# LordTARN1SHED/Image-Restoration-for-Road-Sign-Recognition-in-Autonomous-Driving

Hardware: AMD Instinct MI355X
Metric: images/sec ResUNet fwd+bwd (64x64 GTSRB batch) at 1/2/4/8 MI355X; PSNR parity (higher is better)
Workload: dtype bf16; 1 GPU; cfg3: ResUNet unified train step (dynamic distortion + ToTensor, fwd + L1 + 0.1*VGG16[:16] perceptual + bwd + AdamW), 14_train_unified_advanced.py; global_batch=512, per_gpu_batch=512, parallelism=dp1, hip_graph=True

## Files before the change

image-restoration-for-road-sign-recognition-in-autonomous-driving_amd/csrc/conv_in.hip:

```cpp
#include "common.h"

namespace {

template <typename T>
__global__ void conv_in_fwd_kernel(int n, int h, int w, int cin, int cout,
                                   const float *__restrict__ x, const float *__restrict__ wt,
                                   const float *__restrict__ b, int act, const float *alpha,
                                   T *__restrict__ y) {
  extern __shared__ __attribute__((aligned(16))) float sw[];
  const int kk = cin * 9;
  for (int i = threadIdx.x; i < kk * cout; i += blockDim.x) {
    const int co = i % cout, j = i / cout;
    sw[i] = wt[(long long)co * kk + j];
  }
  for (int i = threadIdx.x; i < cout; i += blockDim.x) sw[kk * cout + i] = b ? b[i] : 0.f;
  __syncthreads();
  const int G = cout / 4;
  const long long P = (long long)n * h * w;
  const float al = alpha ? alpha[0] : 0.f;
  for (long long id = blockIdx.x * (long long)blockDim.x + threadIdx.x; id < P * G;
       id += (long long)gridDim.x * blockDim.x) {
    const int g = (int)(id % G);
    const long long p = id / G;
    const int ww = (int)(p % w);
    const long long nh = p / w;
    const int hh = (int)(nh % h);
    const int nn = (int)(nh / h);
    f32x4 acc = *reinterpret_cast<const f32x4 *>(sw + kk * cout + g * 4);
    for (int ci = 0; ci < cin; ++ci) {
      const float *xp = x + ((long long)nn * cin + ci) * h * w;
#pragma unroll
      for (int t = 0; t < 9; ++t) {
        const int y2 = hh + t / 3 - 1, x2 = ww + t % 3 - 1;
        if (y2 < 0 || y2 >= h || x2 < 0 || x2 >= w) continue;
        const float v = xp[(long long)y2 * w + x2];
        acc += v * *reinterpret_cast<const f32x4 *>(sw + (ci * 9 + t) * cout + g * 4);
      }
    }
    if (act == 1) {
#pragma unroll
      for (int k = 0; k < 4; ++k) acc[k] = fmaxf(acc[k], 0.f);
    } else if (act == 2) {
#pragma unroll
      for (int k = 0; k < 4; ++k) acc[k] = acc[k] > 0.f ? acc[k] : al * acc[k];
    }
    store4<T>(y + p * cout + g * 4, acc);
  }
}

template <typename T>
__global__ void conv_in_wgrad_kernel(int n, int h, int w, int cin, int cout,
                                     const float *__restrict__ x, const T *__restrict__ dy,
                                     float *__restrict__ part, long long px_per_block) {
  __shared__ __attribute__((aligned(16))) float sdy[64][65];
  __shared__ __attribute__((aligned(16))) float spt[64][32];
  const int kk = cin * 9;
  const long long P = (long long)n * h * w;
  const long long pb = blockIdx.x * px_per_block;
  const long long pe = min(P, pb + px_per_block);
  const int co = threadIdx.x & 63, jg = threadIdx.x >> 6;
  double acc[8] = {0, 0, 0, 0, 0, 0, 0, 0};
  for (long long p0 = pb; p0 < pe; p0 += 64) {
    __syncthreads();
    for (int i = threadIdx.x; i < 64 * 64; i += blockDim.x) {
      const int r = i >> 6, c = i & 63;
      const long long p = p0 + r;
      sdy[r][c] = (p < pe && c < cout) ? Elt<T>::load(dy, p * cout + c) : 0.f;
    }
    for (int i = threadIdx.x; i < 64 * 32; i += blockDim.x) {
      const int r = i >> 5, j = i & 31;
      const long long p = p0 + r;
      float v = 0.f;
      if (p < pe) {
        if (j < kk) {
          const int ci = j / 9, t = j % 9;
          const int ww = (int)(p % w);
          const long long nh = p / w;
          const int hh = (int)(nh % h);
          const int nn = (int)(nh / h);
          const int y2 = hh + t / 3 - 1, x2 = ww + t % 3 - 1;
          if (y2 >= 0 && y2 < h && x2 >= 0 && x2 < w)
            v = x[(((long long)nn * cin + ci) * h + y2) * w + x2];
        } else if (j == kk) {
          v = 1.f;
        }
      }
      spt[r][j] = v;
    }
    __syncthreads();
    if (co < cout) {
      float st[8] = {0.f, 0.f, 0.f, 0.f, 0.f, 0.f, 0.f, 0.f};
#pragma unroll 4
      for (int r = 0; r < 64; ++r) {
        const float d = sdy[r][co];
        const f32x4 a0 = *reinterpret_cast<const f32x4 *>(&spt[r][jg * 8]);
        const f32x4 a1 = *reinterpret_cast<const f32x4 *>(&spt[r][jg * 8 + 4]);
#pragma unroll
        for (int k = 0; k < 4; ++k) { st[k] += d * a0[k]; st[4 + k] += d * a1[k]; }
      }
#pragma unroll
      for (int k = 0; k < 8; ++k) acc[k] += st[k];
    }
  }
  if (co < cout) {
#pragma unroll
    for (int k = 0; k < 8; ++k) part[((long long)blockIdx.x * cout + co) * 32 + jg * 8 + k] = (float)acc[k];
  }
}

constexpr int CIA_NPX = 64;
constexpr int CIA_ROW = CIA_NPX + 8;
constexpr int CIA_XROW = 32 + 8;
template <bool REC>
__global__ __launch_bounds__(256, REC ? 4 : 1) void conv_in_wgrad_act_kernel(
    int n, int h, int w, const float *__restrict__ x, const bf16_t *__restrict__ g,
    const bf16_t *__restrict__ t, int act, const float *__restrict__ alpha,
    float *__restrict__ part, long long ppb) {
  __shared__ __attribute__((aligned(16))) u16 gT[64 * CIA_ROW];
  __shared__ __attribute__((aligned(16))) u16 pT[32 * CIA_ROW];
  __shared__ __attribute__((aligned(16))) u16 pX[REC ? CIA_NPX * CIA_XROW : 8];
  __shared__ float red[256];
  const int tid = threadIdx.x, lane = tid & 63, wv = tid >> 6;
  const long long P = (long long)n * h * w, hw = (long long)h * w;
  const long long p0 = blockIdx.x * ppb, p1 = min(P, p0 + ppb);
  const float al = act == 2 ? alpha[0] : 0.f;
  float sa = 0.f;
  f32x4 acc[2] = {f32x4{0.f, 0.f, 0.f, 0.f}, f32x4{0.f, 0.f, 0.f, 0.f}};
  const int lc = tid & 7, lpp = tid >> 3;
  const int bn = lane & 15, bk = lane >> 4;
  const int sj = tid & 63, sg = tid >> 6;
  uint4 rg[2], rt[2] = {};
  float rp[8];
  auto load_step = [&](long long q0) __attribute__((always_inline)) {
#pragma unroll
    for (int j = 0; j < 2; ++j) {
      const long long p = q0 + 2 * lpp + j;
      const bool ok = p < p1;
      const long long e = (ok ? p : p0) * 64 + lc * 8;
      rg[j] = *reinterpret_cast<const uint4 *>(g + e);
      if constexpr (!REC) rt[j] = *reinterpret_cast<const uint4 *>(t + e);
      if (!ok) rg[j] = uint4{0u, 0u, 0u, 0u};
    }
    const long long p = q0 + sj;
    const bool live = p < p1;
    int img = 0, y = 0, xx0 = 0;
    if (live) {
      img = (int)(p / hw);
      const int rem = (int)(p - img * hw);
      y = rem / w;
      xx0 = rem - y * w;
    }
#pragma unroll
    for (int u = 0; u < 8; ++u) {
      const int r = sg + 4 * u;
      float val = 0.f;
      if (r < 27) {
        const int ci = r / 9, ky = (r % 9) / 3, kx = r % 3;
        const int yy = y + ky - 1, xx = xx0 + kx - 1;
        const bool ok = live && yy >= 0 && yy < h && xx >= 0 && xx < w;
        const float vv = x[ok ? (((long long)img * 3 + ci) * h + yy) * w + xx : 0];
        val = ok ? vv : 0.f;
      } else if (r == 27) {
        val = live ? 1.f : 0.f;
      }
      rp[u] = val;
    }
  };
  auto bf = [](uint32_t word, int hi) { return __uint_as_float(hi ? (word & 0xffff0000u) : (word << 16)); };
  bf16x8 fw = {};
  if constexpr (REC) fw = *reinterpret_cast<const bf16x8 *>(t + (wv * 16 + bn) * 32 + bk * 8);
  if (p0 < p1) load_step(p0);
  for (long long q0 = p0; q0 < p1; q0 += CIA_NPX) {
    if constexpr (REC) {
#pragma unroll
      for (int u = 0; u < 8; ++u) {
        const u16 pv = f32_to_bf16(rp[u]);
        pT[(sg + 4 * u) * CIA_ROW + sj] = pv;
        pX[sj * CIA_XROW + sg + 4 * u] = pv;
      }
      __syncthreads();
#pragma unroll
      for (int nb = 0; nb < 4; ++nb) {
        const bf16x8 fp = *reinterpret_cast<const bf16x8 *>(&pX[(nb * 16 + bn) * CIA_XROW + bk * 8]);
        const f32x4 tv = __builtin_amdgcn_mfma_f32_16x16x32_bf16(fw, fp, f32x4{0.f, 0.f, 0.f, 0.f}, 0, 0, 0);
#pragma unroll
        for (int i = 0; i < 4; ++i) gT[(wv * 16 + 4 * bk + i) * CIA_ROW + nb * 16 + bn] = f32_to_bf16(tv[i]);
      }
      __syncthreads();
    }
    u16 v[2][8];
    uint32_t tpair[8];
    if constexpr (REC) {
#pragma unroll
      for (int k = 0; k < 8; ++k)
        tpair[k] = *reinterpret_cast<const uint32_t *>(&gT[(lc * 8 + k) * CIA_ROW + 2 * lpp]);
    }
#pragma unroll
    for (int j = 0; j < 2; ++j) {
      const uint32_t gw[4] = {rg[j].x, rg[j].y, rg[j].z, rg[j].w};
      const uint32_t tw[4] = {rt[j].x, rt[j].y, rt[j].z, rt[j].w};
#pragma unroll
      for (int k = 0; k < 8; ++k) {
        const float gg = bf(gw[k >> 1], k & 1);
        const float tt = REC ? bf(tpair[k], j) : bf(tw[k >> 1], k & 1);
        const float gp = tt > 0.f ? gg : al * gg;
        sa += tt > 0.f ? 0.f : gg * tt;
        v[j][k] = f32_to_bf16(gp);
      }
    }
#pragma unroll
    for (int k = 0; k < 8; ++k)
      *reinterpret_cast<uint32_t *>(&gT[(lc * 8 + k) * CIA_ROW + 2 * lpp]) =
          (uint32_t)v[0][k] | ((uint32_t)v[1][k] << 16);
    if constexpr (!REC) {
#pragma unroll
      for (int u = 0; u < 8; ++u) pT[(sg + 4 * u) * CIA_ROW + sj] = f32_to_bf16(rp[u]);
    }
    __syncthreads();
    if (q0 + CIA_NPX < p1) load_step(q0 + CIA_NPX);
#pragma unroll
    for (int ks = 0; ks < 2; ++ks) {
      const int px = ks * 32 + bk * 8;
      const bf16x8 fa = *reinterpret_cast<const bf16x8 *>(&gT[(wv * 16 + bn) * CIA_ROW + px]);
#pragma unroll
      for (int nb = 0; nb < 2; ++nb) {
        const bf16x8 fb = *reinterpret_cast<const bf16x8 *>(&pT[(nb * 16 + bn) * CIA_ROW + px]);
        acc[nb] = __builtin_amdgcn_mfma_f32_16x16x32_bf16(fa, fb, acc[nb], 0, 0, 0);
      }
    }
    __syncthreads();
  }
  float *pw = part + (long long)blockIdx.x * (64 * 32 + 32);
#pragma unroll
  for (int nb = 0; nb < 2; ++nb)
#pragma unroll
    for (int i = 0; i < 4; ++i) pw[(wv * 16 + 4 * bk + i) * 32 + nb * 16 + bn] = acc[nb][i];
  red[tid] = sa;
  __syncthreads();
  for (int o = 128; o > 0; o >>= 1) {
    if (tid < o) red[tid] += red[tid + o];
    __syncthreads();
  }
  if (tid < 32) pw[64 * 32 + tid] = tid == 0 ? red[0] : 0.f;
}

__global__ void conv_in_wgrad_act_finalize(int chunks, const double *__restrict__ part, float *dw,
                                           float *db, float *dalpha) {
  const int i = blockIdx.x * blockDim.x + threadIdx.x;
  const int cols = 64 * 32 + 32;
  if (i > 64 * 32) return;
  double sv[1] = {0};
  rr_fixed_sum<1>(part + i, cols, chunks, sv);
  const double s = sv[0];
  if (i == 64 * 32) {
    if (dalpha) dalpha[0] = (float)s;
    return;
  }
  const int co = i / 32, j = i % 32;
  if (j < 27) dw[co * 27 + j] = (float)s;
  else if (j == 27 && db) db[co] = (float)s;
}

__global__ void conv_in_wgrad_finalize(int cout, int kk, int blocks, const double *__restrict__ part,
                                       float *dw, float *db) {
  const int i = blockIdx.x * blockDim.x + threadIdx.x;
  if (i >= cout * 32) return;
  const int co = i / 32, j = i % 32;
  if (j > kk) return;
  double sv[1] = {0};
  rr_fixed_sum<1>(part + i, (long long)cout * 32, blocks, sv);
  const double s = sv[0];
  if (j < kk) dw[(long long)co * kk + j] = (float)s;
  else if (db) db[co] = (float)s;
}

template <typename T>
__global__ void conv_in_dgrad_kernel(int n, int h, int w, int cin, int cout,
                                     const T *__restrict__ dy, const float *__restrict__ wt,
                                     float *__restrict__ dx, int accumulate) {
  extern __shared__ __attribute__((aligned(16))) float sw[];
  const int kk = cin * 9;
  for (int i = threadIdx.x; i < kk * cout; i += blockDim.x) {
    const int co = i % cout, j = i / cout;
    const int t = j / cin, ci = j % cin;
    sw[i] = wt[((long long)co * cin + ci) * 9 + t];
  }
  __syncthreads();
  const long long P = (long long)n * h * w;
  for (long long p = blockIdx.x * (long long)blockDim.x + threadIdx.x; p < P;
       p += (long long)gridDim.x * blockDim.x) {
    const int ww = (int)(p % w);
    const long long nh = p / w;
    const int hh = (int)(nh % h);
    const int nn = (int)(nh / h);
    float acc[4] = {0.f, 0.f, 0.f, 0.f};
    for (int t = 0; t < 9; ++t) {
      const int ky = t / 3, kx = t % 3;
      const int y2 = hh - ky + 1, x2 = ww - kx + 1;
      if (y2 < 0 || y2 >= h || x2 < 0 || x2 >= w) continue;
      const T *dp = dy + (((long long)nn * h + y2) * w + x2) * cout;
      for (int c = 0; c < cout; c += 4) {
        const f32x4 d = load4<T>(dp + c);
        for (int ci = 0; ci < cin && ci < 4; ++ci) {
          const f32x4 wv = *reinterpret_cast<const f32x4 *>(sw + (t * cin + ci) * cout + c);
          acc[ci] += d[0] * wv[0] + d[1] * wv[1] + d[2] * wv[2] + d[3] * wv[3];
        }
      }
    }
    for (int ci = 0; ci < cin && ci < 4; ++ci) {
      const long long o = (((long long)nn * cin + ci) * h + hh) * w + ww;
      dx[o] = accumulate ? dx[o] + acc[ci] : acc[ci];
    }
  }
}

template <typename T>
__global__ void im2col3_kernel(int n, int h, int w, int cin, int kpad, const float *__restrict__ x,
                               T *__restrict__ col) {
  const int G = kpad / 4;
  const long long total = (long long)n * h * w * G;
  const int kk = cin * 9;
  for (long long i = blockIdx.x * (long long)blockDim.x + threadIdx.x; i < total;
       i += (long long)gridDim.x * blockDim.x) {
    const int g = (int)(i % G);
    const long long p = i / G;
    const int ww = (int)(p % w);
    const long long nh = p / w;
    const int hh = (int)(nh % h);
    const int nn = (int)(nh / h);
    f32x4 v;
#pragma unroll
    for (int e = 0; e < 4; ++e) {
      const int j = g * 4 + e;
      float val = 0.f;
      if (j < kk) {
        const int ci = j / 9, t = j - (j / 9) * 9;
        const int y2 = hh + t / 3 - 1, x2 = ww + t % 3 - 1;
        if (y2 >= 0 && y2 < h && x2 >= 0 && x2 < w)
          val = x[(((long long)nn * cin + ci) * h + y2) * w + x2];
      } else if (j == kk) {
        val = 1.f;
      }
      v[e] = val;
    }
    store4<T>(col + p * kpad + g * 4, v);
  }
}

__global__ __launch_bounds__(256) void conv_in_mfma_kernel(int n, int h, int w,
                                                           const float *__restrict__ x,
                                                           const bf16_t *__restrict__ wp, int act,
                                                           const float *__restrict__ alpha,
                                                           bf16_t *__restrict__ y_pre,
                                                           bf16_t *__restrict__ y_act) {
  constexpr int SR = 68;
  __shared__ __attribute__((aligned(16))) float stg[4][32 * SR];
  const int lane = threadIdx.x & 63, wv = threadIdx.x >> 6;
  const long long hw = (long long)h * w;
  const long long P = (long long)n * hw;
  const long long p0 = ((long long)blockIdx.x * 4 + wv) * 64;
  if (p0 >= P) return;
  const int fr = lane & 15, q = lane >> 4;
  bf16x8 fa[4];
#pragma unroll
  for (int mi = 0; mi < 4; ++mi)
    fa[mi] = *reinterpret_cast<const bf16x8 *>(wp + (mi * 16 + fr) * 32 + q * 8);
  const int hwi = h * w;
  int kofs[8], kdy[8], kdx[8];
  bool ktap[8], kone[8];
#pragma unroll
  for (int j = 0; j < 8; ++j) {
    const int k = q * 8 + j;
    const int ci = k / 9, t = k - (k / 9) * 9;
    kdy[j] = t / 3 - 1;
    kdx[j] = t % 3 - 1;
    kofs[j] = ci * hwi + kdy[j] * w + kdx[j];
    ktap[j] = k < 27;
    kone[j] = k == 27;
  }
  const int Pi = (int)P;
  const __amdgpu_buffer_rsrc_t xr = __builtin_amdgcn_make_buffer_rsrc(
      const_cast<float *>(x), 0, (int)(3 * P * 4), 0x00020000);
  const int pw0 = (int)p0;
// ... 217 lines not shown
```

image-restoration-for-road-sign-recognition-in-autonomous-driving_amd/csrc/conv_out.hip:

```cpp
#include "common.h"

namespace {

template <typename T>
__global__ void conv_out_fwd_kernel(int n, int h, int w, int cin, int cout, const T *__restrict__ x,
                                    const float *__restrict__ wt, const float *__restrict__ b,
                                    float *__restrict__ y) {
  extern __shared__ __attribute__((aligned(16))) float sw[];
  for (int i = threadIdx.x; i < cin * cout; i += blockDim.x) sw[i] = wt[i];
  __syncthreads();
  const long long P = (long long)n * h * w;
  const long long hw = (long long)h * w;
  for (long long p = blockIdx.x * (long long)blockDim.x + threadIdx.x; p < P;
       p += (long long)gridDim.x * blockDim.x) {
    float acc[4] = {0.f, 0.f, 0.f, 0.f};
    const T *xp = x + p * cin;
    for (int c = 0; c < cin; c += 4) {
      const f32x4 v = load4<T>(xp + c);
      for (int co = 0; co < cout && co < 4; ++co) {
        const f32x4 wv = *reinterpret_cast<const f32x4 *>(sw + co * cin + c);
        acc[co] += v[0] * wv[0] + v[1] * wv[1] + v[2] * wv[2] + v[3] * wv[3];
      }
    }
    const long long nn = p / hw, r = p % hw;
    for (int co = 0; co < cout && co < 4; ++co)
      y[(nn * cout + co) * hw + r] = acc[co] + (b ? b[co] : 0.f);
  }
}

template <typename T>
__global__ void conv_out_bwd_kernel(int n, int h, int w, int cin, int cout,
                                    const float *__restrict__ dy, const T *__restrict__ x,
                                    const float *__restrict__ wt, T *__restrict__ dx, int mask_relu,
                                    float *__restrict__ part, long long px_per_block) {
  __shared__ float red[4][64][4];
  __shared__ float redb[4][4];
  const int ci = threadIdx.x & 63, row = threadIdx.x >> 6;
  const long long hw = (long long)h * w;
  const long long P = (long long)n * hw;
  const long long pb = blockIdx.x * px_per_block;
  const long long pe = min(P, pb + px_per_block);
  float wv[4] = {0.f, 0.f, 0.f, 0.f};
  for (int co = 0; co < cout; ++co) wv[co] = ci < cin ? wt[co * cin + ci] : 0.f;
  float sw[4] = {0.f, 0.f, 0.f, 0.f}, sb[4] = {0.f, 0.f, 0.f, 0.f};
  for (long long p = pb + row; p < pe; p += 4) {
    const long long nn = p / hw, r = p - nn * hw;
    float d[4] = {0.f, 0.f, 0.f, 0.f};
    for (int co = 0; co < cout; ++co) d[co] = dy[(nn * cout + co) * hw + r];
    if (ci < cin) {
      const float xv = Elt<T>::load(x, p * cin + ci);
      float g = 0.f;
      for (int co = 0; co < cout; ++co) {
        g += d[co] * wv[co];
        sw[co] += d[co] * xv;
      }
      if (mask_relu && !(xv > 0.f)) g = 0.f;
      if (dx) Elt<T>::store(dx, p * cin + ci, g);
    }
    for (int co = 0; co < cout; ++co) sb[co] += d[co];
  }
  for (int co = 0; co < 4; ++co) red[row][ci][co] = sw[co];
  if (ci == 0)
    for (int co = 0; co < 4; ++co) redb[row][co] = sb[co];
  __syncthreads();
  if (row == 0 && ci < cin)
    for (int co = 0; co < cout; ++co)
      part[((long long)blockIdx.x * (cout + 1) + co) * cin + ci] =
          red[0][ci][co] + red[1][ci][co] + red[2][ci][co] + red[3][ci][co];
  if (threadIdx.x < cout) {
    const int co = threadIdx.x;
    part[((long long)blockIdx.x * (cout + 1) + cout) * cin + co] =
        redb[0][co] + redb[1][co] + redb[2][co] + redb[3][co];
  }
}

template <typename T, int COUT>
__global__ __launch_bounds__(256) void conv_out_bwd64_kernel(
    int n, int h, int w, const float *__restrict__ dy, const T *__restrict__ x,
    const float *__restrict__ wt, T *__restrict__ dx, int mask_relu, float *__restrict__ part,
    long long px_per_block) {
  constexpr int CIN = 64;
  __shared__ float red[4][COUT + 1][CIN];
  const int cg = threadIdx.x & 7, pl = threadIdx.x >> 3;
  const long long hw = (long long)h * w;
  const long long P = (long long)n * hw;
  const long long pb = blockIdx.x * px_per_block;
  const long long pe = min(P, pb + px_per_block);
  float wv[COUT][8];
#pragma unroll
  for (int co = 0; co < COUT; ++co)
#pragma unroll
    for (int j = 0; j < 8; ++j) wv[co][j] = wt[co * CIN + cg * 8 + j];
  float sw[COUT][8], sb[COUT];
#pragma unroll
  for (int co = 0; co < COUT; ++co) {
    sb[co] = 0.f;
#pragma unroll
    for (int j = 0; j < 8; ++j) sw[co][j] = 0.f;
  }
  auto one = [&](long long p) __attribute__((always_inline)) {
    const long long nn = p / hw, r = p - nn * hw;
    float d[COUT];
#pragma unroll
    for (int co = 0; co < COUT; ++co) d[co] = dy[(nn * COUT + co) * hw + r];
    const T *xp = x + p * CIN + cg * 8;
    const f32x4 x0 = load4<T>(xp), x1 = load4<T>(xp + 4);
    const float xv[8] = {x0[0], x0[1], x0[2], x0[3], x1[0], x1[1], x1[2], x1[3]};
    float g[8];
#pragma unroll
    for (int j = 0; j < 8; ++j) {
      float t = 0.f;
#pragma unroll
      for (int co = 0; co < COUT; ++co) {
        t += d[co] * wv[co][j];
        sw[co][j] += d[co] * xv[j];
      }
      g[j] = (mask_relu && !(xv[j] > 0.f)) ? 0.f : t;
    }
#pragma unroll
    for (int co = 0; co < COUT; ++co) sb[co] += d[co];
    if (dx) store8<T>(dx + p * CIN + cg * 8, f32x4{g[0], g[1], g[2], g[3]}, f32x4{g[4], g[5], g[6], g[7]});
  };
  long long p = pb + pl;
  for (; p + 32 < pe; p += 64) {
    one(p);
    one(p + 32);
  }
  if (p < pe) one(p);
#pragma unroll
  for (int co = 0; co < COUT; ++co) {
#pragma unroll
    for (int j = 0; j < 8; ++j) {
      float v = sw[co][j];
      v += __shfl_xor(v, 8, 64);
      v += __shfl_xor(v, 16, 64);
      v += __shfl_xor(v, 32, 64);
      sw[co][j] = v;
    }
    float v = sb[co];
    v += __shfl_xor(v, 8, 64);
    v += __shfl_xor(v, 16, 64);
    v += __shfl_xor(v, 32, 64);
    sb[co] = v;
  }
  const int wv_ = threadIdx.x >> 6, lane = threadIdx.x & 63;
  if (lane < 8) {
#pragma unroll
    for (int co = 0; co < COUT; ++co) {
#pragma unroll
      for (int j = 0; j < 8; ++j) red[wv_][co][cg * 8 + j] = sw[co][j];
      if (cg == 0) red[wv_][COUT][co] = sb[co];
    }
  }
  __syncthreads();
  for (int i = threadIdx.x; i < COUT * CIN + COUT; i += 256) {
    const int co = i / CIN, ci = i - co * CIN;
    part[(long long)blockIdx.x * (COUT + 1) * CIN + i] =
        red[0][co][ci] + red[1][co][ci] + red[2][co][ci] + red[3][co][ci];
  }
}

template <typename T, int COUT, bool REC = false>
__global__ __launch_bounds__(256) void conv_out_bwd64_bnred_kernel(
    int n, int h, int w, const float *__restrict__ dy, const T *__restrict__ x,
    const float *__restrict__ wt, const T *__restrict__ t0, const float *__restrict__ mean0,
    const float *__restrict__ inv0, const T *__restrict__ t1, const float *__restrict__ mean1,
    const float *__restrict__ inv1, float *__restrict__ part, float *__restrict__ bnpart,
    long long px_per_block, const float *__restrict__ aff_s = nullptr,
    const float *__restrict__ aff_b = nullptr) {
  constexpr int CIN = 64;
  __shared__ float red[4][COUT + 1][CIN];
  __shared__ float bred[4][CIN][3];
  const int cg = threadIdx.x & 7, pl = threadIdx.x >> 3;
  const long long hw = (long long)h * w;
  const long long P = (long long)n * hw;
  const long long pb = blockIdx.x * px_per_block;
  const long long pe = min(P, pb + px_per_block);
  float wv[COUT][8], m0[8], i0[8], m1[8], i1[8];
#pragma unroll
  for (int j = 0; j < 8; ++j) {
#pragma unroll
    for (int co = 0; co < COUT; ++co) wv[co][j] = wt[co * CIN + cg * 8 + j];
    m0[j] = mean0[cg * 8 + j]; i0[j] = inv0[cg * 8 + j];
    m1[j] = mean1[cg * 8 + j]; i1[j] = inv1[cg * 8 + j];
  }
  __shared__ __attribute__((aligned(16))) float faff[REC ? 4 * CIN : 4];
  if constexpr (REC) {
    faff[threadIdx.x] = threadIdx.x < 2 * CIN ? aff_s[threadIdx.x] : aff_b[threadIdx.x - 2 * CIN];
    __syncthreads();
  }
  float sw[COUT][8], sb[COUT], bs[3][8];
#pragma unroll
  for (int co = 0; co < COUT; ++co) {
    sb[co] = 0.f;
#pragma unroll
    for (int j = 0; j < 8; ++j) sw[co][j] = 0.f;
  }
#pragma unroll
  for (int j = 0; j < 8; ++j) { bs[0][j] = 0.f; bs[1][j] = 0.f; bs[2][j] = 0.f; }
  auto one = [&](long long p) __attribute__((always_inline)) {
    const long long nn = p / hw, r = p - nn * hw;
    float d[COUT];
#pragma unroll
    for (int co = 0; co < COUT; ++co) d[co] = dy[(nn * COUT + co) * hw + r];
    const long long e = p * CIN + cg * 8;
    f32x4 x0, x1, a0, a1, b0, b1;
    load8<T>(t0 + e, a0, a1);
    load8<T>(t1 + e, b0, b1);
    if constexpr (REC) {
      int o = cg * 8;
      asm volatile("" : "+v"(o));
      const f32x4 *fa = reinterpret_cast<const f32x4 *>(faff + o);
      f32x4 v0 = a0 * fa[0] + fa[32], v1 = a1 * fa[1] + fa[33];
      f32x4 q0 = b0 * fa[16] + fa[48], q1 = b1 * fa[17] + fa[49];
      v0 += q0;
      v1 += q1;
#pragma unroll
      for (int k = 0; k < 4; ++k) {
        x0[k] = Elt<T>::round(fmaxf(v0[k], 0.f));
        x1[k] = Elt<T>::round(fmaxf(v1[k], 0.f));
      }
    } else {
      load8<T>(x + e, x0, x1);
    }
    const float xv[8] = {x0[0], x0[1], x0[2], x0[3], x1[0], x1[1], x1[2], x1[3]};
    const float ta[8] = {a0[0], a0[1], a0[2], a0[3], a1[0], a1[1], a1[2], a1[3]};
    const float tb[8] = {b0[0], b0[1], b0[2], b0[3], b1[0], b1[1], b1[2], b1[3]};
#pragma unroll
    for (int j = 0; j < 8; ++j) {
      float t = 0.f;
#pragma unroll
      for (int co = 0; co < COUT; ++co) {
        t += d[co] * wv[co][j];
        sw[co][j] += d[co] * xv[j];
      }
      const float gm = xv[j] > 0.f ? Elt<T>::round(t) : 0.f;
      bs[0][j] += gm;
      bs[1][j] += gm * ((ta[j] - m0[j]) * i0[j]);
      bs[2][j] += gm * ((tb[j] - m1[j]) * i1[j]);
    }
#pragma unroll
    for (int co = 0; co < COUT; ++co) sb[co] += d[co];
  };
  long long p = pb + pl;
  for (; p + 32 < pe; p += 64) {
    one(p);
    one(p + 32);
  }
  if (p < pe) one(p);
  auto lanes8 = [](float v) __attribute__((always_inline)) {
    v += __shfl_xor(v, 8, 64);
    v += __shfl_xor(v, 16, 64);
    v += __shfl_xor(v, 32, 64);
    return v;
  };
#pragma unroll
  for (int co = 0; co < COUT; ++co) {
#pragma unroll
    for (int j = 0; j < 8; ++j) sw[co][j] = lanes8(sw[co][j]);
    sb[co] = lanes8(sb[co]);
  }
#pragma unroll
  for (int k = 0; k < 3; ++k)
#pragma unroll
    for (int j = 0; j < 8; ++j) bs[k][j] = lanes8(bs[k][j]);
  const int wv_ = threadIdx.x >> 6, lane = threadIdx.x & 63;
  if (lane < 8) {
#pragma unroll
    for (int co = 0; co < COUT; ++co) {
#pragma unroll
      for (int j = 0; j < 8; ++j) red[wv_][co][cg * 8 + j] = sw[co][j];
      if (cg == 0) red[wv_][COUT][co] = sb[co];
    }
#pragma unroll
    for (int j = 0; j < 8; ++j)
#pragma unroll
      for (int k = 0; k < 3; ++k) bred[wv_][cg * 8 + j][k] = bs[k][j];
  }
  __syncthreads();
  for (int i = threadIdx.x; i < COUT * CIN + COUT; i += 256) {
    const int co = i / CIN, ci = i - co * CIN;
    part[(long long)blockIdx.x * (COUT + 1) * CIN + i] =
        red[0][co][ci] + red[1][co][ci] + red[2][co][ci] + red[3][co][ci];
  }
  if (threadIdx.x < CIN * 3) {
    const int c = threadIdx.x / 3, k = threadIdx.x - c * 3;
    bnpart[(long long)blockIdx.x * CIN * 3 + threadIdx.x] =
        bred[0][c][k] + bred[1][c][k] + bred[2][c][k] + bred[3][c][k];
  }
}

constexpr int TCO_D = 2;
__global__ __launch_bounds__(256) void tail_conv_out_kernel(
    int P, int hw, int cout, const bf16_t *__restrict__ x, const float *__restrict__ scale,
    const float *__restrict__ shift, const bf16_t *__restrict__ res, const float *__restrict__ rs,
    const float *__restrict__ rb, const bf16_t *__restrict__ wp, const float *__restrict__ bias,
    bf16_t *__restrict__ y, float *__restrict__ out) {
  const int lane = threadIdx.x & 63;
  const int wv = __builtin_amdgcn_readfirstlane(threadIdx.x >> 6);
  const int fr = lane & 15, fq = lane >> 4;
  const int nblk = (P + 15) >> 4;
  const int gw = blockIdx.x * 4 + wv, NWT = gridDim.x * 4;
  bf16x8 wr[2];
  f32x4 s[2][2], b[2][2], qs[2][2], qb[2][2];
#pragma unroll
  for (int kb = 0; kb < 2; ++kb) {
    bf16x8 v = {};
    if (fr < cout) v = *reinterpret_cast<const bf16x8 *>(wp + fr * 64 + kb * 32 + fq * 8);
    wr[kb] = v;
#pragma unroll
    for (int hf = 0; hf < 2; ++hf) {
      const int c = kb * 32 + fq * 8 + 4 * hf;
      s[kb][hf] = *reinterpret_cast<const f32x4 *>(scale + c);
      b[kb][hf] = *reinterpret_cast<const f32x4 *>(shift + c);
      qs[kb][hf] = *reinterpret_cast<const f32x4 *>(rs + c);
      qb[kb][hf] = *reinterpret_cast<const f32x4 *>(rb + c);
    }
  }
  float bv[4];
#pragma unroll
  for (int j = 0; j < 4; ++j) bv[j] = j < cout ? bias[j] : 0.f;
  struct Blk {
    uint4 t[2], r[2];
  };
  auto load_blk = [&](int bi, Blk &bk) __attribute__((always_inline)) {
    const int p = min(bi * 16 + fr, P - 1);
    const long long e = (long long)p * 64 + fq * 8;
#pragma unroll
    for (int kb = 0; kb < 2; ++kb) {
      bk.t[kb] = *reinterpret_cast<const uint4 *>(x + e + kb * 32);
      bk.r[kb] = *reinterpret_cast<const uint4 *>(res + e + kb * 32);
    }
  };
  auto unpack = [](uint4 r, f32x4 &lo, f32x4 &hi) __attribute__((always_inline)) {
    lo[0] = __uint_as_float(r.x << 16); lo[1] = __uint_as_float(r.x & 0xffff0000u);
    lo[2] = __uint_as_float(r.y << 16); lo[3] = __uint_as_float(r.y & 0xffff0000u);
    hi[0] = __uint_as_float(r.z << 16); hi[1] = __uint_as_float(r.z & 0xffff0000u);
    hi[2] = __uint_as_float(r.w << 16); hi[3] = __uint_as_float(r.w & 0xffff0000u);
  };
  auto run = [&](const Blk &bk, int bi) __attribute__((always_inline)) {
    const int p = bi * 16 + fr;
    const bool live = p < P;
    f32x4 acc = f32x4{0.f, 0.f, 0.f, 0.f};
#pragma unroll
    for (int kb = 0; kb < 2; ++kb) {
      f32x4 v0, v1, q0, q1;
      unpack(bk.t[kb], v0, v1);
      unpack(bk.r[kb], q0, q1);
      v0 = v0 * s[kb][0] + b[kb][0];
      v1 = v1 * s[kb][1] + b[kb][1];
      q0 = q0 * qs[kb][0] + qb[kb][0];
      q1 = q1 * qs[kb][1] + qb[kb][1];
      v0 += q0;
      v1 += q1;
#pragma unroll
      for (int k = 0; k < 4; ++k) { v0[k] = fmaxf(v0[k], 0.f); v1[k] = fmaxf(v1[k], 0.f); }
      u16x8 r;
      r[0] = f32_to_bf16(v0[0]); r[1] = f32_to_bf16(v0[1]); r[2] = f32_to_bf16(v0[2]); r[3] = f32_to_bf16(v0[3]);
      r[4] = f32_to_bf16(v1[0]); r[5] = f32_to_bf16(v1[1]); r[6] = f32_to_bf16(v1[2]); r[7] = f32_to_bf16(v1[3]);
      if (y && live) *reinterpret_cast<u16x8 *>(y + (long long)p * 64 + kb * 32 + fq * 8) = r;
      acc = __builtin_amdgcn_mfma_f32_16x16x32_bf16(wr[kb], __builtin_bit_cast(bf16x8, r), acc, 0, 0, 0);
    }
    if (live && fq == 0) {
      const int n = p / hw, rem = p - n * hw;
#pragma unroll
      for (int j = 0; j < 4; ++j)
        if (j < cout) out[((long long)n * cout + j) * hw + rem] = acc[j] + bv[j];
    }
  };
  for (int b0 = gw; b0 < nblk; b0 += TCO_D * NWT) {
    Blk bk[TCO_D];
#pragma unroll
    for (int j = 0; j < TCO_D; ++j) load_blk(min(b0 + j * NWT, nblk - 1), bk[j]);
#pragma unroll
    for (int j = 0; j < TCO_D; ++j)
      if (b0 + j * NWT < nblk) run(bk[j], b0 + j * NWT);
  }
}

__global__ void conv_out_bwd_finalize(int cin, int cout, int blocks, const double *__restrict__ part,
                                      float *dw, float *db) {
  const int i = blockIdx.x * blockDim.x + threadIdx.x;
  if (i >= cout * cin + cout) return;
  double s = 0;
  if (i < cout * cin) {
    double sv[1] = {0};
    rr_fixed_sum<1>(part + i, (long long)(cout + 1) * cin, blocks, sv);
    s = sv[0];
    if (dw) dw[i] = (float)s;
  } else {
    const int co = i - cout * cin;
    double sv[1] = {0};
    rr_fixed_sum<1>(part + (long long)cout * cin + co, (long long)(cout + 1) * cin, blocks, sv);
    s = sv[0];
    if (db) db[co] = (float)s;
  }
}

}

extern "C" int rr_conv_out_fwd(int dtype, int n, int h, int w, int cin, int cout, const void *x,
                               const float *wt, const float *b, float *y, rr_stream stream) {
// ... 153 lines not shown
```

Baseline: 36940 images/sec.

## Double-buffer conv_in wgrad LDS tiles and software-prefetch conv_out bwd pixel loads

The first-layer weight-gradient kernel now gives each thread one pixel. It recomputes the fused activation input in registers with MFMA instead of staging it through an extra LDS array, and it replaces per-step div/mod with an incremental position walker. The gT/pT tiles are double-buffered, which drops one barrier per iteration, and launch bounds are raised to 4 waves for both variants. In conv_out backward, loads for the next two pixels are issued before the current ones are used, and an incremental plane walker replaces the per-pixel division. The changes trade more registers and LDS for better latency hiding, and the MFMA operand remapping must exactly match the previous layout.

```diff
diff --git a/image-restoration-for-road-sign-recognition-in-autonomous-driving_amd/csrc/conv_in.hip b/image-restoration-for-road-sign-recognition-in-autonomous-driving_amd/csrc/conv_in.hip
--- a/image-restoration-for-road-sign-recognition-in-autonomous-driving_amd/csrc/conv_in.hip
+++ b/image-restoration-for-road-sign-recognition-in-autonomous-driving_amd/csrc/conv_in.hip
@@ -110,15 +110,13 @@
 
 constexpr int CIA_NPX = 64;
 constexpr int CIA_ROW = CIA_NPX + 8;
-constexpr int CIA_XROW = 32 + 8;
 template <bool REC>
-__global__ __launch_bounds__(256, REC ? 4 : 1) void conv_in_wgrad_act_kernel(
+__global__ __launch_bounds__(256, 4) void conv_in_wgrad_act_kernel(
     int n, int h, int w, const float *__restrict__ x, const bf16_t *__restrict__ g,
     const bf16_t *__restrict__ t, int act, const float *__restrict__ alpha,
     float *__restrict__ part, long long ppb) {
-  __shared__ __attribute__((aligned(16))) u16 gT[64 * CIA_ROW];
-  __shared__ __attribute__((aligned(16))) u16 pT[32 * CIA_ROW];
-  __shared__ __attribute__((aligned(16))) u16 pX[REC ? CIA_NPX * CIA_XROW : 8];
+  __shared__ __attribute__((aligned(16))) u16 gT[2][64 * CIA_ROW];
+  __shared__ __attribute__((aligned(16))) u16 pT[2][32 * CIA_ROW];
   __shared__ float red[256];
   const int tid = threadIdx.x, lane = tid & 63, wv = tid >> 6;
   const long long P = (long long)n * h * w, hw = (long long)h * w;
@@ -126,109 +124,114 @@
   const float al = act == 2 ? alpha[0] : 0.f;
   float sa = 0.f;
   f32x4 acc[2] = {f32x4{0.f, 0.f, 0.f, 0.f}, f32x4{0.f, 0.f, 0.f, 0.f}};
-  const int lc = tid & 7, lpp = tid >> 3;
   const int bn = lane & 15, bk = lane >> 4;
-  const int sj = tid & 63, sg = tid >> 6;
+  const int px = wv * 16 + bn;
+  long long kofs[8];
+  int kdy[8], kdx[8];
+  bool ktap[8], kone[8];
+#pragma unroll
+  for (int j = 0; j < 8; ++j) {
+    const int k = bk * 8 + j;
+    const int ci = k / 9, tp = k - ci * 9;
+    kdy[j] = tp / 3 - 1;
+    kdx[j] = tp % 3 - 1;
+    kofs[j] = ci * hw + kdy[j] * (long long)w + kdx[j];
+    ktap[j] = k < 27;
+    kone[j] = k == 27;
+  }
+  long long pq = p0 + px, xo = 0;
+  int py = 0, pxx = 0;
+  if (pq < p1) {
+    const long long img = pq / hw;
+    const int rem = (int)(pq - img * hw);
+    py = rem / w;
+    pxx = rem - py * w;
+    xo = img * 3 * hw + rem;
+  }
+  auto next_pos = [&]() __attribute__((always_inline)) {
+    pq += CIA_NPX;
+    xo += CIA_NPX;
+    pxx += CIA_NPX;
+    while (pxx >= w) {
+      pxx -= w;
+      if (++py == h) { py = 0; xo += 2 * hw; }
+    }
+  };
   uint4 rg[2], rt[2] = {};
   float rp[8];
-  auto load_step = [&](long long q0) __attribute__((always_inline)) {
-#pragma unroll
-    for (int j = 0; j < 2; ++j) {
-      const long long p = q0 + 2 * lpp + j;
-      const bool ok = p < p1;
-      const long long e = (ok ? p : p0) * 64 + lc * 8;
-      rg[j] = *reinterpret_cast<const uint4 *>(g + e);
-      if constexpr (!REC) rt[j] = *reinterpret_cast<const uint4 *>(t + e);
-      if (!ok) rg[j] = uint4{0u, 0u, 0u, 0u};
-    }
-    const long long p = q0 + sj;
-    const bool live = p < p1;
-    int img = 0, y = 0, xx0 = 0;
-    if (live) {
-      img = (int)(p / hw);
-      const int rem = (int)(p - img * hw);
-      y = rem / w;
-      xx0 = rem - y * w;
-    }
-#pragma unroll
-    for (int u = 0; u < 8; ++u) {
-      const int r = sg + 4 * u;
-      float val = 0.f;
-      if (r < 27) {
-        const int ci = r / 9, ky = (r % 9) / 3, kx = r % 3;
-        const int yy = y + ky - 1, xx = xx0 + kx - 1;
-        const bool ok = live && yy >= 0 && yy < h && xx >= 0 && xx < w;
-        const float vv = x[ok ? (((long long)img * 3 + ci) * h + yy) * w + xx : 0];
-        val = ok ? vv : 0.f;
-      } else if (r == 27) {
-        val = live ? 1.f : 0.f;
-      }
-      rp[u] = val;
+  auto load_step = [&]() __attribute__((always_inline)) {
+    const bool live = pq < p1;
+    const long long e = (live ? pq : p0) * 64 + bk * 8;
+#pragma unroll
+    for (int c = 0; c < 2; ++c) {
+      rg[c] = *reinterpret_cast<const uint4 *>(g + e + c * 32);
+      if constexpr (!REC) rt[c] = *reinterpret_cast<const uint4 *>(t + e + c * 32);
+      if (!live) rg[c] = uint4{0u, 0u, 0u, 0u};
+    }
+#pragma unroll
+    for (int j = 0; j < 8; ++j) {
+      const int yy = py + kdy[j], xx = pxx + kdx[j];
+      const bool ok = live && ktap[j] && (unsigned)yy < (unsigned)h && (unsigned)xx < (unsigned)w;
+      const float vv = x[ok ? xo + kofs[j] : 0];
+      rp[j] = ok ? vv : (kone[j] && live ? 1.f : 0.f);
     }
   };
   auto bf = [](uint32_t word, int hi) { return __uint_as_float(hi ? (word & 0xffff0000u) : (word << 16)); };
-  bf16x8 fw = {};
-  if constexpr (REC) fw = *reinterpret_cast<const bf16x8 *>(t + (wv * 16 + bn) * 32 + bk * 8);
-  if (p0 < p1) load_step(p0);
-  for (long long q0 = p0; q0 < p1; q0 += CIA_NPX) {
-    if constexpr (REC) {
-#pragma unroll
-      for (int u = 0; u < 8; ++u) {
-        const u16 pv = f32_to_bf16(rp[u]);
-        pT[(sg + 4 * u) * CIA_ROW + sj] = pv;
-        pX[sj * CIA_XROW + sg + 4 * u] = pv;
-      }
-      __syncthreads();
-#pragma unroll
-      for (int nb = 0; nb < 4; ++nb) {
-        const bf16x8 fp = *reinterpret_cast<const bf16x8 *>(&pX[(nb * 16 + bn) * CIA_XROW + bk * 8]);
-        const f32x4 tv = __builtin_amdgcn_mfma_f32_16x16x32_bf16(fw, fp, f32x4{0.f, 0.f, 0.f, 0.f}, 0, 0, 0);
-#pragma unroll
-        for (int i = 0; i < 4; ++i) gT[(wv * 16 + 4 * bk + i) * CIA_ROW + nb * 16 + bn] = f32_to_bf16(tv[i]);
-      }
-      __syncthreads();
-    }
-    u16 v[2][8];
-    uint32_t tpair[8];
-    if constexpr (REC) {
-#pragma unroll
-      for (int k = 0; k < 8; ++k)
-        tpair[k] = *reinterpret_cast<const uint32_t *>(&gT[(lc * 8 + k) * CIA_ROW + 2 * lpp]);
-    }
-#pragma unroll
-    for (int j = 0; j < 2; ++j) {
-      const uint32_t gw[4] = {rg[j].x, rg[j].y, rg[j].z, rg[j].w};
-      const uint32_t tw[4] = {rt[j].x, rt[j].y, rt[j].z, rt[j].w};
+  bf16x8 fw[2][2] = {};
+  if constexpr (REC) {
+#pragma unroll
+    for (int c = 0; c < 2; ++c)
+#pragma unroll
+      for (int hf = 0; hf < 2; ++hf)
+        fw[c][hf] = *reinterpret_cast<const bf16x8 *>(
+            t + (c * 32 + 8 * (bn >> 2) + 4 * hf + (bn & 3)) * 32 + bk * 8);
+  }
+  if (p0 < p1) load_step();
+  int buf = 0;
+  for (long long q0 = p0; q0 < p1; q0 += CIA_NPX, buf ^= 1) {
+    u16 *gTb = gT[buf], *pTb = pT[buf];
+    u16x8 pv;
+#pragma unroll
+    for (int j = 0; j < 8; ++j) {
+      pv[j] = f32_to_bf16(rp[j]);
+      pTb[(bk * 8 + j) * CIA_ROW + px] = pv[j];
+    }
+#pragma unroll
+    for (int c = 0; c < 2; ++c) {
+      const uint32_t gw[4] = {rg[c].x, rg[c].y, rg[c].z, rg[c].w};
+      const uint32_t tw[4] = {rt[c].x, rt[c].y, rt[c].z, rt[c].w};
+      float tr[8];
+      if constexpr (REC) {
+#pragma unroll
+        for (int hf = 0; hf < 2; ++hf) {
+          const f32x4 tv = __builtin_amdgcn_mfma_f32_16x16x32_bf16(
+              fw[c][hf], __builtin_bit_cast(bf16x8, pv), f32x4{0.f, 0.f, 0.f, 0.f}, 0, 0, 0);
+#pragma unroll
+          for (int i = 0; i < 4; ++i) tr[4 * hf + i] = bf16_to_f32(f32_to_bf16(tv[i]));
+        }
+      }
 #pragma unroll
       for (int k = 0; k < 8; ++k) {
         const float gg = bf(gw[k >> 1], k & 1);
-        const float tt = REC ? bf(tpair[k], j) : bf(tw[k >> 1], k & 1);
+        const float tt = REC ? tr[k] : bf(tw[k >> 1], k & 1);
         const float gp = tt > 0.f ? gg : al * gg;
         sa += tt > 0.f ? 0.f : gg * tt;
-        v[j][k] = f32_to_bf16(gp);
-      }
-    }
-#pragma unroll
-    for (int k = 0; k < 8; ++k)
-      *reinterpret_cast<uint32_t *>(&gT[(lc * 8 + k) * CIA_ROW + 2 * lpp]) =
-          (uint32_t)v[0][k] | ((uint32_t)v[1][k] << 16);
-    if constexpr (!REC) {
-#pragma unroll
-      for (int u = 0; u < 8; ++u) pT[(sg + 4 * u) * CIA_ROW + sj] = f32_to_bf16(rp[u]);
+        gTb[(c * 32 + bk * 8 + k) * CIA_ROW + px] = f32_to_bf16(gp);
+      }
     }
     __syncthreads();
-    if (q0 + CIA_NPX < p1) load_step(q0 + CIA_NPX);
+    next_pos();
+    if (q0 + CIA_NPX < p1) load_step();
 #pragma unroll
     for (int ks = 0; ks < 2; ++ks) {
-      const int px = ks * 32 + bk * 8;
-      const bf16x8 fa = *reinterpret_cast<const bf16x8 *>(&gT[(wv * 16 + bn) * CIA_ROW + px]);
+      const int kp = ks * 32 + bk * 8;
+      const bf16x8 fa = *reinterpret_cast<const bf16x8 *>(&gTb[(wv * 16 + bn) * CIA_ROW + kp]);
 #pragma unroll
       for (int nb = 0; nb < 2; ++nb) {
-        const bf16x8 fb = *reinterpret_cast<const bf16x8 *>(&pT[(nb * 16 + bn) * CIA_ROW + px]);
+        const bf16x8 fb = *reinterpret_cast<const bf16x8 *>(&pTb[(nb * 16 + bn) * CIA_ROW + kp]);
         acc[nb] = __builtin_amdgcn_mfma_f32_16x16x32_bf16(fa, fb, acc[nb], 0, 0, 0);
       }
     }
-    __syncthreads();
   }
   float *pw = part + (long long)blockIdx.x * (64 * 32 + 32);
 #pragma unroll
diff --git a/image-restoration-for-road-sign-recognition-in-autonomous-driving_amd/csrc/conv_out.hip b/image-restoration-for-road-sign-recognition-in-autonomous-driving_amd/csrc/conv_out.hip
--- a/image-restoration-for-road-sign-recognition-in-autonomous-driving_amd/csrc/conv_out.hip
+++ b/image-restoration-for-road-sign-recognition-in-autonomous-driving_amd/csrc/conv_out.hip
@@ -74,6 +74,68 @@
   }
 }
 
+template <typename T> struct Raw8;
+template <> struct Raw8<bf16_t> {
+  uint4 v;
+  __device__ __forceinline__ void load(const bf16_t *p) { v = *reinterpret_cast<const uint4 *>(p); }
+  __device__ __forceinline__ void get(f32x4 &a, f32x4 &b) const {
+    a[0] = __uint_as_float(v.x << 16); a[1] = __uint_as_float(v.x & 0xffff0000u);
+    a[2] = __uint_as_float(v.y << 16); a[3] = __uint_as_float(v.y & 0xffff0000u);
+    b[0] = __uint_as_float(v.z << 16); b[1] = __uint_as_float(v.z & 0xffff0000u);
+    b[2] = __uint_as_float(v.w << 16); b[3] = __uint_as_float(v.w & 0xffff0000u);
+  }
+};
+template <> struct Raw8<float> {
+  f32x4 lo, hi;
+  __device__ __forceinline__ void load(const float *p) {
+    lo = *reinterpret_cast<const f32x4 *>(p);
+    hi = *reinterpret_cast<const f32x4 *>(p + 4);
+  }
+  __device__ __forceinline__ void get(f32x4 &a, f32x4 &b) const { a = lo; b = hi; }
+};
+
+struct NoRaw8 {
+  template <typename P> __device__ __forceinline__ void load(P) {}
+  __device__ __forceinline__ void get(f32x4 &, f32x4 &) const {}
+};
+
+template <int COUT> struct PlaneWalk {
+  long long p, o;
+  long long r, hw;
+  __device__ __forceinline__ PlaneWalk(long long p_, long long hw_) : p(p_), hw(hw_) {
+    const long long nn = p_ / hw_;
+    r = p_ - nn * hw_;
+    o = nn * COUT * hw_ + r;
+  }
+  __device__ __forceinline__ void step32() {
+    p += 32; r += 32; o += 32;
+    while (r >= hw) { r -= hw; o += (COUT - 1) * hw; }
+  }
+};
+
+template <typename L, typename F, typename U>
+__device__ __forceinline__ void pixel_pairs_ahead(int cnt, F &&fetch, U &&use) {
+  L cur[2];
+  if (cnt > 0) fetch(cur[0]);
+  if (cnt > 1) fetch(cur[1]);
+  int i = 0;
+  for (; i + 3 < cnt; i += 2) {
+    L nxt[2];
+    fetch(nxt[0]);
+    fetch(nxt[1]);
+    use(cur[0]);
+    use(cur[1]);
+    cur[0] = nxt[0];
+    cur[1] = nxt[1];
+  }
+  if (i < cnt) use(cur[0]);
+  if (i + 1 < cnt) use(cur[1]);
+  if (i + 2 < cnt) {
+    fetch(cur[0]);
+    use(cur[0]);
+  }
+}
+
 template <typename T, int COUT>
 __global__ __launch_bounds__(256) void conv_out_bwd64_kernel(
     int n, int h, int w, const float *__restrict__ dy, const T *__restrict__ x,
@@ -98,13 +160,26 @@
 #pragma unroll
     for (int j = 0; j < 8; ++j) sw[co][j] = 0.f;
   }
-  auto one = [&](long long p) __attribute__((always_inline)) {
-    const long long nn = p / hw, r = p - nn * hw;
+  struct Px {
+    long long p;
     float d[COUT];
-#pragma unroll
-    for (int co = 0; co < COUT; ++co) d[co] = dy[(nn * COUT + co) * hw + r];
-    const T *xp = x + p * CIN + cg * 8;
-    const f32x4 x0 = load4<T>(xp), x1 = load4<T>(xp + 4);
+    Raw8<T> x;
+  };
+  const long long pf = pb + pl;
+  const int cnt = pf < pe ? (int)((pe - pf + 31) >> 5) : 0;
+  PlaneWalk<COUT> wk(pf, cnt ? hw : 1);
+  auto fetch = [&](Px &L) __attribute__((always_inline)) {
+    L.p = wk.p;
+#pragma unroll
+    for (int co = 0; co < COUT; ++co) L.d[co] = dy[wk.o + co * hw];
+    L.x.load(x + wk.p * CIN + cg * 8);
+    wk.step32();
+  };
+  auto one = [&](const Px &L) __attribute__((always_inline)) {
+    const long long p = L.p;
+    const float *d = L.d;
+    f32x4 x0, x1;
+    L.x.get(x0, x1);
     const float xv[8] = {x0[0], x0[1], x0[2], x0[3], x1[0], x1[1], x1[2], x1[3]};
     float g[8];
 #pragma unroll
@@ -121,12 +196,7 @@
     for (int co = 0; co < COUT; ++co) sb[co] += d[co];
     if (dx) store8<T>(dx + p * CIN + cg * 8, f32x4{g[0], g[1], g[2], g[3]}, f32x4{g[4], g[5], g[6], g[7]});
   };
-  long long p = pb + pl;
-  for (; p + 32 < pe; p += 64) {
-    one(p);
-    one(p + 32);
-  }
-  if (p < pe) one(p);
+  pixel_pairs_ahead<Px>(cnt, fetch, one);
 #pragma unroll
   for (int co = 0; co < COUT; ++co) {
 #pragma unroll
@@ -198,15 +268,28 @@
   }
 #pragma unroll
   for (int j = 0; j < 8; ++j) { bs[0][j] = 0.f; bs[1][j] = 0.f; bs[2][j] = 0.f; }
-  auto one = [&](long long p) __attribute__((always_inline)) {
-    const long long nn = p / hw, r = p - nn * hw;
+  struct Px {
     float d[COUT];
-#pragma unroll
-    for (int co = 0; co < COUT; ++co) d[co] = dy[(nn * COUT + co) * hw + r];
-    const long long e = p * CIN + cg * 8;
+    Raw8<T> a, b;
+    std::conditional_t<REC, NoRaw8, Raw8<T>> x;
+  };
+  const long long pf = pb + pl;
+  const int cnt = pf < pe ? (int)((pe - pf + 31) >> 5) : 0;
+  PlaneWalk<COUT> wk(pf, cnt ? hw : 1);
+  auto fetch = [&](Px &L) __attribute__((always_inline)) {
+#pragma unroll
+    for (int co = 0; co < COUT; ++co) L.d[co] = dy[wk.o + co * hw];
+    const long long e = wk.p * CIN + cg * 8;
+    L.a.load(t0 + e);
+    L.b.load(t1 + e);
+    if constexpr (!REC) L.x.load(x + e);
+    wk.step32();
+  };
+  auto one = [&](const Px &L) __attribute__((always_inline)) {
+    const float *d = L.d;
     f32x4 x0, x1, a0, a1, b0, b1;
-    load8<T>(t0 + e, a0, a1);
-    load8<T>(t1 + e, b0, b1);
+    L.a.get(a0, a1);
+    L.b.get(b0, b1);
     if constexpr (REC) {
       int o = cg * 8;
       asm volatile("" : "+v"(o));
@@ -221,7 +304,7 @@
         x1[k] = Elt<T>::round(fmaxf(v1[k], 0.f));
       }
     } else {
-      load8<T>(x + e, x0, x1);
+      L.x.get(x0, x1);
     }
     const float xv[8] = {x0[0], x0[1], x0[2], x0[3], x1[0], x1[1], x1[2], x1[3]};
     const float ta[8] = {a0[0], a0[1], a0[2], a0[3], a1[0], a1[1], a1[2], a1[3]};
@@ -242,12 +325,7 @@
 #pragma unroll
     for (int co = 0; co < COUT; ++co) sb[co] += d[co];
   };
-  long long p = pb + pl;
-  for (; p + 32 < pe; p += 64) {
-    one(p);
-    one(p + 32);
-  }
-  if (p < pe) one(p);
+  pixel_pairs_ahead<Px>(cnt, fetch, one);
   auto lanes8 = [](float v) __attribute__((always_inline)) {
     v += __shfl_xor(v, 8, 64);
     v += __shfl_xor(v, 16, 64);
```

After: 36890 images/sec. No clear change (-0.1%).
